# kennethsoh/IE-ACHE

Measured on AMD Instinct MI355X. Metric: bootstrapped gate ops/sec; encrypted 32-bit MUL/sec, higher is better.
Workload: dtype int32; 1 GPU; 16-bit ADD, batch 4096 ciphertext pairs, 1xMI355X (level-batched bootstraps); circuit=add16, batch_per_gpu=4096, bootstraps_per_expr=80, levels=48, params=n=630 N=1024 k=1 l=3 Bgbit=7 ks_t=8 ks_basebit=2, parallelism=batch-sharded x1, kernel=w1x64-radix8-onelimb, overlap_streams=2, rccl_ranks=0

## Files before the change

ie-ache_amd/__init__.py:

```python
from .evaluator import (
    CIRC_ADD, CIRC_SUB, CIRC_RSUB, CIRC_MUL, CIRC_MULADD, CIRC_ADD_KS, CIRC_SUB_KS, CIRC_RSUB_KS, CIRC_MUL_WALLACE,
    GATE_AND, GATE_XOR, GATE_OR, GATE_NAND, GATE_MUX, circ_chain,
    GATE_NOR, GATE_XNOR, GATE_ANDNY, GATE_ANDYN, GATE_ORNY, GATE_ORYN, GATE_TYPES, FALSE, TRUE, NOT, Netlist, CompiledNetlist,
    CircuitInfo, Context, IeacheError, Params, Stats, build_library, circuit_info, circuit_level_cap, circuit_simulate,
    default_params, device_count, debug_forward_path, lib, library_path,
    GATE_MAJ3, GATE_XOR3, CIRC_ADD_FA, CIRC_SUB_FA, CIRC_RSUB_FA, CIRC_MUL_FA, circuit_gate_count,
    PBS_NO_KEYSWITCH, PBS_TLWE_POLYS, PBS_ACCUMULATOR, PBS_MULTI_MAX_FACTORS, Group, GROUP_MAX_DEVICES, Job,
    TgswSet, Automaton, AUTOMATON_MAX_STATES, AUTOMATON_MAX_STEPS, automaton_tables, LUT_TREE_MAX_DEPTH, ROTATE_MAX_STEPS, LUT_READ_NO_KEYSWITCH,
    FFT_FORWARD_FORMS, FFT_INVERSE_FORMS, FFT_PAIRED_FORMS, TWIDDLE_ENTRIES,
)
from . import tools
from . import netlists
from . import automata
from . import programs
from .programs import WordProgram, Register, netlist_export
from .programs import FAMILY_REFERENCE, FAMILY_KOGGE_STONE, FAMILY_CARRY_SAVE, FAMILY_FULL_ADDER
from .compute import compute, compute_final, FAILURE_SIZE
```

ie-ache_amd/csrc/blind_rotate_w64.hip:

```cpp
#include "blind_rotate_w64.h"

#include <cstdio>
#include <algorithm>
#include <stdexcept>
#include <type_traits>
#include <vector>

#include "br_step.h"
#include "fft_probe.h"
#include "mix_plan.h"

namespace ieache {
namespace w64 {

using namespace dev;

namespace {

__global__ __launch_bounds__(64) void k_bk_to_spectrum_w64(const Torus32* bk_raw, double2* bkf) {
    __shared__ __align__(16) double2 sT[kTile];
    __shared__ __align__(16) double2 sTw[kTwElems];
    const int lane = threadIdx.x;
    build_twiddles(sTw, lane, 64);
    __syncthreads();
// ... 169 lines not shown
#pragma unroll 1
        for (int q = 1; q < L; q++) digit_row(q, std::false_type{});
        fft512_inverse_pair<true>(s[0], s[1], sT, lane, R);
#pragma unroll
        for (int r = 0; r < 8; r++) {
            double unused = 0.0;
            const uint32_t l0 = round_coef(s[0][r].x, untwist_gain(r), false, unused), l1 = round_coef(s[0][r].y, untwist_gain(r), false, unused);
            const uint32_t h0 = round_coef(s[1][r].x, untwist_gain(r), false, unused), h1 = round_coef(s[1][r].y, untwist_gain(r), false, unused);
            const int32_t j = 64 * r + lane;
            accw[j] = (int32_t)((uint32_t)accw[j] + l0 + (h0 << 16));
            accw[j + kM] = (int32_t)((uint32_t)accw[j + kM] + l1 + (h1 << 16));
        }
    }
    __syncthreads();
    finish_slice<128>(ext, item, acc, gacc, tid);
}


template <int L, int BGBIT, int GUARD, bool DIAG = false, int G = kW1Gates, int XLANE = 2>
__global__ __launch_bounds__(64 * G, 2) void k_blind_rotate_w1b(DevKeys K, const double2* __restrict__ bkf1,
                                                                       const uint16_t* __restrict__ st_bara, int32_t nb,
                                                                       int32_t* st_acc, int64_t items, int32_t i0, int32_t i1,
                                                                       Torus32* ext, unsigned* guard,
                                                                       const double2* __restrict__ gtw, unsigned long long* diag = nullptr) {
    extern __shared__ __align__(16) unsigned char smem[];
    int32_t* acc_all = reinterpret_cast<int32_t*>(smem);
    double2* sT_all = reinterpret_cast<double2*>(smem + (size_t)G * 2 * kN * 4);
    double2* sTw = sT_all + G * kTile;
    const int tid = threadIdx.x, lane = tid & 63;
    const int wave = __builtin_amdgcn_readfirstlane(tid >> 6);
    double2* sT = sT_all + wave * kTile;
    int32_t* acc = acc_all + wave * 2 * kN;
    const int64_t item = (int64_t)blockIdx.x * G + wave;
    static_assert(XLANE == 1 || XLANE == 2, "the forward transforms' lane-high transpose: v_cndmask pairs (1) or the exchange form (2)");
    using Roots = typename std::conditional<XLANE == 2, LaneRootsExchange, LaneRootsResident>::type;
    load_twiddles(sTw, gtw, tid, 64 * G);
    __syncthreads();
    if (item >= items) return;
    const Roots R = make_roots<Roots>(sTw, lane);
    const int plane = XLANE == 2 ? xl_pi(lane) : lane;
    const uint16_t* __restrict__ bara = st_bara + (size_t)item * nb;
    int32_t* gacc = st_acc + (size_t)item * 2 * kN;
    {
        const int4* src = reinterpret_cast<const int4*>(gacc);
        int4* dst = reinterpret_cast<int4*>(acc);
#pragma unroll
        for (int r = 0; r < 8; r++) dst[64 * r + lane] = src[64 * r + lane];
    }
    wave_sync();

    constexpr uint32_t halfBg = 1u << (BGBIT - 1);
    uint32_t dec_offset = 0;
#pragma unroll
    for (int q = 1; q <= L; q++) dec_offset += halfBg << (32 - q * BGBIT);
    float dev_maxf = 0.0f;
    constexpr int kRowBytes = 2 * kM * (int)sizeof(double2), kStepBytes = 2 * L * kRowBytes;
    const __amdgpu_buffer_rsrc_t bk_rsrc = bk_resource(bkf1, K.n, kStepBytes);
    const int lane16 = bk_lane_offset(lane);
    const unsigned char* accb = reinterpret_cast<const unsigned char*>(acc_all);
    const uint32_t pb0 = (uint32_t)wave * (2 * kN * 4);

    unsigned long long tsum[8] = {0, 0, 0, 0, 0, 0, 0, 0}, tlast = 0;
    if (DIAG) tlast = stamp();
    const int32_t my_a = lane_amounts(bara, i0, i1, lane);
#pragma unroll 1
    for (int32_t i = i0; i < i1; i++) {
        const int32_t a = __builtin_amdgcn_readlane(my_a, i - i0);
        if (a == 0) continue;
        const int bki = i * kStepBytes;
        double2 s[2][8];
        uint32_t v0[8], v1[8];
        double dev_max = 0.0;
        const uint32_t jb4 = ((uint32_t)(plane - a) & (2 * kN - 1)) << 2;
        auto decompose = [&](const uint32_t pb) {
            const int32_t* accp = reinterpret_cast<const int32_t*>(accb + pb);
            decompose_rotated(v0, v1, accb, accp, pb, jb4, plane, dec_offset);
        };
        auto digit_row = [&](const int sh, const int brow, auto first) {
            constexpr bool FIRST = decltype(first)::value;
            double2 x[8], bA[8], bB[8];
            auto request_a = [&]() { load_bk_block(bA, bk_rsrc, lane16, brow); };
            digits_to_double2<BGBIT>(x, v0, v1, sh);
            __builtin_amdgcn_sched_barrier(0);
            stamp_phase<DIAG>(tsum, tlast, 1);
            fft512_forward<true, XLANE>(x, sT, lane, R, request_a);
            stamp_phase<DIAG>(tsum, tlast, 2);
            load_bk_block(bB, bk_rsrc, lane16, brow + kRowBytes / 2);
            __builtin_amdgcn_sched_barrier(0);
#pragma unroll
            for (int k = 0; k < 8; k++) s[0][k] = mac<FIRST>(s[0][k], x[k], bA[k]);
#pragma unroll
            for (int k = 0; k < 8; k++) s[1][k] = mac<FIRST>(s[1][k], x[k], bB[k]);
            stamp_phase<DIAG>(tsum, tlast, 3);
        };
        decompose(pb0);
        stamp_phase<DIAG>(tsum, tlast, 0);
        digit_row(32 - BGBIT, bki, std::true_type{});
#pragma unroll 1
        for (int row = 1; row < L; row++) digit_row(32 - (row + 1) * BGBIT, bki + row * kRowBytes, std::false_type{});
        decompose(pb0 + 4096u);
        stamp_phase<DIAG>(tsum, tlast, 0);
#pragma unroll 1
        for (int row = L; row < 2 * L; row++) digit_row(32 - (row - L + 1) * BGBIT, bki + row * kRowBytes, std::false_type{});
        fft512_inverse_pair<true>(s[0], s[1], sT, lane, R);
        stamp_phase<DIAG>(tsum, tlast, 4);
#pragma unroll
        for (int c = 0; c < 2; c++) {
            uint32_t* accc = reinterpret_cast<uint32_t*>(acc) + c * kN;
#pragma unroll
            for (int r = 0; r < 8; r++) {
                const bool watched = GUARD == 1 || (GUARD == 2 && (r & 3) == 0);
                const uint32_t d0 = round_coef(s[c][r].x, untwist_gain(r), watched, dev_max), d1 = round_coef(s[c][r].y, untwist_gain(r), watched, dev_max);
                const int32_t j = 64 * r + lane;
                __hip_atomic_fetch_add(&accc[j], d0, __ATOMIC_RELAXED, __HIP_MEMORY_SCOPE_WAVEFRONT);
                __hip_atomic_fetch_add(&accc[j + kM], d1, __ATOMIC_RELAXED, __HIP_MEMORY_SCOPE_WAVEFRONT);
            }
        }
        if (GUARD) dev_maxf = fmaxf(dev_maxf, (float)dev_max);
        wave_sync();
        stamp_phase<DIAG>(tsum, tlast, 5);
    }
    if (DIAG && diag && lane == 0) {
#pragma unroll
        for (int t = 0; t < 8; t++) atomicAdd(&diag[(wave & 1) * 8 + t], tsum[t]);
    }
    int elane = lane;
    asm volatile("" : "+v"(elane));
    if (GUARD) publish_guard((double)dev_maxf, guard, elane);
    finish_slice<64>(ext, item, acc, gacc, elane);
}

template <int L, int BGBIT, int G = kW1Gates>
__global__ __launch_bounds__(64 * G, 2) void k_blind_rotate_x1(DevKeys K, const double2* __restrict__ bkf,
                                                                      const uint16_t* __restrict__ st_bara, int32_t nb,
                                                                      int32_t* st_acc, int64_t items, int32_t i0, int32_t i1,
                                                                      Torus32* ext, const double2* __restrict__ gtw) {
    extern __shared__ __align__(16) unsigned char smem[];
    int32_t* acc_all = reinterpret_cast<int32_t*>(smem);
    double2* sT_all = reinterpret_cast<double2*>(smem + (size_t)G * 2 * kN * 4);
    double2* sTw = sT_all + G * kTile;
    const int tid = threadIdx.x, lane = tid & 63;
    const int wave = __builtin_amdgcn_readfirstlane(tid >> 6);
    double2* sT = sT_all + wave * kTile;
    int32_t* acc = acc_all + wave * 2 * kN;
    const int64_t item = (int64_t)blockIdx.x * G + wave;
    load_twiddles(sTw, gtw, tid, 64 * G);
    __syncthreads();
    if (item >= items) return;
    const LaneRoots R = make_roots(sTw, lane);
    const uint16_t* __restrict__ bara = st_bara + (size_t)item * nb;
    int32_t* gacc = st_acc + (size_t)item * 2 * kN;
    {
        const int4* src = reinterpret_cast<const int4*>(gacc);
        int4* dst = reinterpret_cast<int4*>(acc);
#pragma unroll
        for (int r = 0; r < 8; r++) dst[64 * r + lane] = src[64 * r + lane];
    }
    wave_sync();

    constexpr uint32_t halfBg = 1u << (BGBIT - 1);
    uint32_t dec_offset = 0;
#pragma unroll
// ... 618 lines not shown
        char what[96];
        snprintf(what, sizeof what, "%s<%d,%d> (br_variant %d, %d gates per workgroup)", br_variant(v.number)->name, PS::L, PS::BGBIT, (int)v.number, v.gates);
        allow_dynamic_lds_once(grant, (const void*)kernel, v.allow, what);
    }
    hipLaunchKernelGGL(kernel, dim3((unsigned)((s.items + v.gates - 1) / v.gates)), dim3(v.threads == kTwoLWaves ? 128 * PS::L : v.threads),
                       v.lds(PS::L, s.nb, v.gates), s.stream, args...);
}
template <class PS, class... P>
static void launch_row(PS ps, const LaunchRow& v, const Slice& s, void (*kernel)(P...), typename as_is<P>::type... args) {
    launch_row_granted(ps, v, s, granted(v, PS::index), kernel, args...);
}
template <int XLANE>
static void go_w2(const LaunchRow& v, const Slice& s) {
    with_param_set(s.l, [&](auto ps) {
        launch_row(ps, v, s, k_blind_rotate_w2<ps.L, ps.BGBIT, XLANE>, s.K, s.t.bkf, s.st_bara, s.nb, s.st_acc, s.i0, s.i1, s.ext, s.t.twiddles);
    });
}
template <int G>
static void go_x1(const LaunchRow& v, const Slice& s) {
    with_param_set(s.l, [&](auto ps) {
        launch_row(ps, v, s, k_blind_rotate_x1<ps.L, ps.BGBIT, G>, s.K, s.t.bkf, s.st_bara, s.nb, s.st_acc, s.items, s.i0, s.i1, s.ext, s.t.twiddles);
    });
}
template <bool DIAG, int LIMBS>
static void go_wide(const LaunchRow& v, const Slice& s) {
    with_param_set(s.l, [&](auto ps) {
        launch_row(ps, v, s, k_blind_rotate_wide<ps.L, ps.BGBIT, DIAG, LIMBS>, s.K, LIMBS == 2 ? s.t.bkf : s.t.bkf1, s.st_bara, s.nb, s.st_acc,
                   s.i0, s.i1, s.ext, DIAG ? s.t.diag : nullptr, s.t.twiddles, LIMBS == 2 ? nullptr : s.t.guard);
    });
}
template <int GUARD, bool DIAG = false, int G = kW1Gates>
static void go_w1b(const LaunchRow& v, const Slice& s) {
    with_param_set(s.l, [&](auto ps) {
        constexpr int XL = (DIAG && ps.L == 2) ? 1 : 2;
        if constexpr (GUARD == 2 && !DIAG) {
            if (probe::w1b_forward_path() == 1) {
                static LdsGrant partner;
                launch_row_granted(ps, v, s, partner, k_blind_rotate_w1b<ps.L, ps.BGBIT, GUARD, DIAG, G, 1>, s.K, s.t.bkf1, s.st_bara, s.nb, s.st_acc,
                                   s.items, s.i0, s.i1, s.ext, s.t.guard, s.t.twiddles, nullptr);
                return;
            }
        }
        launch_row(ps, v, s, k_blind_rotate_w1b<ps.L, ps.BGBIT, GUARD, DIAG, G, XL>, s.K, s.t.bkf1, s.st_bara, s.nb, s.st_acc, s.items, s.i0, s.i1,
                   s.ext, s.t.guard, s.t.twiddles, DIAG ? s.t.diag : nullptr);
    });
}
template <int GUARD>
static void go_w2r(const LaunchRow& v, const Slice& s) {
    with_param_set(s.l, [&](auto ps) {
        launch_row(ps, v, s, k_blind_rotate_w2r<ps.L, ps.BGBIT, GUARD>, s.K, s.t.bkf1, s.st_bara, s.nb, s.st_acc, s.i0, s.i1, s.ext, s.t.guard, s.t.twiddles);
    });
}
template <int GUARD>
static void go_w4r(const LaunchRow& v, const Slice& s) {
    with_param_set(s.l, [&](auto ps) {
        launch_row(ps, v, s, k_blind_rotate_w4r<ps.L, ps.BGBIT, GUARD>, s.K, s.t.bkf1, s.st_bara, s.nb, s.st_acc, s.i0, s.i1, s.ext, s.t.guard, s.t.twiddles,
                   s.flip);
    });
}
template <int GUARD>
static void go_wide4(const LaunchRow& v, const Slice& s) {
    with_param_set(s.l, [&](auto ps) {
        launch_row(ps, v, s, k_blind_rotate_wide4<ps.L, ps.BGBIT, GUARD>, s.K, s.t.bkf1, s.st_bara, s.nb, s.st_acc, s.i0, s.i1, s.ext, s.t.guard, s.t.twiddles);
    });
}

constexpr size_t kAccBytes = (size_t)2 * kN * 4, kCuLds = 160 * 1024;
constexpr size_t lds_bytes_w1(int wg_gates) { return (size_t)(wg_gates * kTile + kTwElems) * sizeof(double2) + (size_t)wg_gates * 2 * kN * 4; }
static size_t lds_w1(int, int32_t, int gates) { return lds_bytes_w1(gates); }
static size_t lds_w2(int, int32_t, int) { return (size_t)(2 * kTile + kTwElems) * sizeof(double2) + kAccBytes; }
static size_t lds_w4(int, int32_t, int) { return (size_t)(4 * kTile + 2 * 8 * 64 + kTwElems) * sizeof(double2) + kAccBytes; }
static size_t lds_wide(int L, int32_t nb, int) { return (size_t)(2 * L * kTile + kTwElems) * sizeof(double2) + kAccBytes + (size_t)nb * 2; }
static size_t lds_wide4(int L, int32_t nb, int) { return (size_t)((2 * L + 4) * kTile + kTwElems) * sizeof(double2) + kAccBytes + (size_t)nb * 2; }

// ... 164 lines not shown
```

ie-ache_amd/csrc/br_step.h:

```cpp
#pragma once
#include "device_common.h"
#include "fft512.h"

namespace ieache {
namespace w64 {
namespace {

using namespace dev;

constexpr int kW1Gates = 4;
constexpr float kGuardLimit = 0.0625f;
__device__ __forceinline__ void publish_guard(double dev_max, unsigned* guard, int lane) {
    float m = (float)dev_max;
#pragma unroll
    for (int o = 32; o >= 1; o >>= 1) m = fmaxf(m, __shfl_xor(m, o, 64));
    if (lane == 0) {
        const unsigned bits = __float_as_uint(m);
        if (bits > __builtin_nontemporal_load(&guard[1])) atomicMax(&guard[1], bits);
        if (m > kGuardLimit) atomicAdd(&guard[0], 1u);
    }
}

template <int NT>
__device__ __forceinline__ void copy_acc(int32_t* to, const int32_t* from, int tid) {
    const int4* src = reinterpret_cast<const int4*>(from);
    int4* dst = reinterpret_cast<int4*>(to);
#pragma unroll
    for (int r = 0; r < 2 * kN / 4 / NT; r++) dst[NT * r + tid] = src[NT * r + tid];
}
template <int NT>
__device__ __forceinline__ void copy_acc_strided(int32_t* to, const int32_t* from, int tid) {
    const int4* src = reinterpret_cast<const int4*>(from);
    int4* dst = reinterpret_cast<int4*>(to);
    for (int idx = tid; idx < 2 * kN / 4; idx += NT) dst[idx] = src[idx];
}
template <int NT>
__device__ __forceinline__ void finish_slice(Torus32* ext, int64_t item, const int32_t* acc, int32_t* gacc, int tid) {
    if (ext) {
        Torus32* u = ext + (size_t)item * (kN + 4);
        for (int32_t j = tid; j <= kN; j += NT)
            u[j] = j == 0 ? acc[0] : (j == kN ? acc[kN] : (int32_t)(0u - (uint32_t)acc[kN - j]));
    } else {
        const int4* src = reinterpret_cast<const int4*>(acc);
        int4* dst = reinterpret_cast<int4*>(gacc);
#pragma unroll
        for (int r = 0; r < 2 * kN / 4 / NT; r++) dst[NT * r + tid] = src[NT * r + tid];
    }
}

__device__ __forceinline__ int32_t lane_amounts(const uint16_t* __restrict__ bara, int32_t i, int32_t i1, int lane) {
    return (i + lane < i1) ? (int32_t)bara[i + lane] : 0;
}

__device__ __forceinline__ __amdgpu_buffer_rsrc_t bk_resource(const double2* bkf, int32_t n, int step_bytes) {
    return __builtin_amdgcn_make_buffer_rsrc(const_cast<double2*>(bkf), (short)0, n * step_bytes, 0x00020000);
}
__device__ __forceinline__ int bk_lane_offset(int lane) { return lane * (int)sizeof(double2); }

template <int L, int BGBIT>
__device__ __forceinline__ uint32_t decomposition_offset() {
    constexpr uint32_t halfBg = 1u << (BGBIT - 1);
    uint32_t dec_offset = 0;
#pragma unroll
    for (int q = 1; q <= L; q++) dec_offset += halfBg << (32 - q * BGBIT);
    return dec_offset;
}
template <int BGBIT>
__device__ __forceinline__ int32_t signed_digit(uint32_t v, int sh) {
    return __builtin_amdgcn_sbfe((int32_t)v, sh, BGBIT);
}
template <int BGBIT>
__device__ __forceinline__ void digits_to_double2(double2 (&x)[8], const uint32_t (&v0)[8], const uint32_t (&v1)[8], int sh) {
#pragma unroll
    for (int r = 0; r < 8; r++) {
        const int32_t e0 = signed_digit<BGBIT>(v0[r], sh), e1 = signed_digit<BGBIT>(v1[r], sh);
        x[r] = make_double2((double)e0, (double)e1);
    }
}

__device__ __forceinline__ void decompose_rotated(uint32_t (&v0)[8], uint32_t (&v1)[8], const unsigned char* accb, const int32_t* accp,
                                                  uint32_t pb, uint32_t jb4, int lane, uint32_t dec_offset) {
#pragma unroll
    for (int r = 0; r < 8; r++) {
        const uint32_t t = jb4 + 256u * r;
        const uint32_t o0 = (t & 4092u) | pb, o1 = o0 ^ 2048u;
        const int32_t m0 = __builtin_amdgcn_sbfe((int32_t)t, 12, 1), m1 = __builtin_amdgcn_sbfe((int32_t)(t + 2048u), 12, 1);
        const uint32_t rv0 = *reinterpret_cast<const uint32_t*>(accb + o0), rv1 = *reinterpret_cast<const uint32_t*>(accb + o1);
        const uint32_t pv0 = (uint32_t)accp[64 * r + lane], pv1 = (uint32_t)accp[64 * r + lane + kM];
        v0[r] = ((rv0 ^ (uint32_t)m0) + ((dec_offset - pv0) - (uint32_t)m0)) ^ dec_offset;
        v1[r] = ((rv1 ^ (uint32_t)m1) + ((dec_offset - pv1) - (uint32_t)m1)) ^ dec_offset;
    }
}

template <bool FIRST>
__device__ __forceinline__ double2 mac(double2 s, double2 x, double2 b) {
    return FIRST ? cmulx<false>(x, b) : make_double2(fma(x.x, b.x, fma(-x.y, b.y, s.x)), fma(x.x, b.y, fma(x.y, b.x, s.y)));
}
template <bool FIRST>
__device__ __forceinline__ void mac_row(double2 (&s)[8], const double2 (&x)[8], const double2 (&b)[8]) {
#pragma unroll
    for (int k = 0; k < 8; k++) s[k] = mac<FIRST>(s[k], x[k], b[k]);
}

template <int BGBIT, bool FIRST>
__device__ __forceinline__ void digit_row_two_limb(double2 (&s)[4][8], const uint32_t (&v0)[8], const uint32_t (&v1)[8], int sh,
                                                   __amdgpu_buffer_rsrc_t bk_rsrc, int lane16, int brow, double2* sT, int lane, const LaneRoots& R) {
    constexpr int kBlockBytes = kM * (int)sizeof(double2);
    double2 x[8], bA[8], bB[8];
    digits_to_double2<BGBIT>(x, v0, v1, sh);
    __builtin_amdgcn_sched_barrier(0);
    auto req = [&]() { load_bk_block(bA, bk_rsrc, lane16, brow); };
    fft512_forward<true, 1, decltype(req), true>(x, sT, lane, R, req);
    load_bk_block(bB, bk_rsrc, lane16, brow + kBlockBytes);
    __builtin_amdgcn_sched_barrier(0);
    mac_row<FIRST>(s[0], x, bA);
    __builtin_amdgcn_sched_barrier(0);
    load_bk_block(bA, bk_rsrc, lane16, brow + 2 * kBlockBytes);
    __builtin_amdgcn_sched_barrier(0);
    mac_row<FIRST>(s[1], x, bB);
    __builtin_amdgcn_sched_barrier(0);
    load_bk_block(bB, bk_rsrc, lane16, brow + 3 * kBlockBytes);
    __builtin_amdgcn_sched_barrier(0);
    mac_row<FIRST>(s[2], x, bA);
    mac_row<FIRST>(s[3], x, bB);
}
// ... 52 lines not shown
```

ie-ache_amd/csrc/capi.cpp:

```cpp
#include "../../include/ieache.h"

#include <cerrno>
#include <cstdio>
#include <cstdlib>
#include <cstring>
#include <initializer_list>
#include <memory>
#include <mutex>
#include <new>
#include <string>
#include <vector>

#include "br_plan.h"
#include "circuit.h"
#include "circuit_cache.h"
#include "cloud_run.h"
#include "cmux.h"
#include "codec.h"
#include "daemon.h"
#include "evaluator.h"
#include "fft_probe.h"
#include "group.h"
#include "group_run.h"
#include "mix_plan.h"
// ... 1371 lines not shown
}

int ieache_debug_twiddles(ieache_ctx* ctx, int which, double* out) {
    return guarded([&] {
        if (!ctx || !out) return fail(IEACHE_EINVAL, "null argument");
        ctx->eval->debug_twiddles(which, out);
        return 0;
    });
}

int ieache_debug_fft512(ieache_ctx* ctx, int form, size_t count, const double* in, double* out) {
    return guarded([&] {
        if (!ctx || !in || !out) return fail(IEACHE_EINVAL, "null argument");
        ctx->eval->debug_fft512(form, count, in, out);
        return 0;
    });
}

int ieache_debug_spectrum(ieache_ctx* ctx, int which, size_t first, size_t count, double* out) {
    return guarded([&] {
        if (!ctx || !out) return fail(IEACHE_EINVAL, "null argument");
        ctx->eval->debug_spectrum(which, first, count, out);
        return 0;
    });
}

int ieache_debug_forward_path(int xlane) {
    return guarded([&] {
        probe::set_w1b_forward_path(xlane);
        return 0;
    });
}

struct ieache_group {
    std::unique_ptr<DeviceGroup> g;
    bool precheck = true;
    ieache_ctx* member(size_t m) const { return g->member(m); }
    size_t size() const { return g->size(); }
};

extern "C++" {
namespace {
struct MemberFailure {
    size_t member;
    int rc;
    std::string message;
};
template <class Call>
int group_call(ieache_group* grp, size_t count, ieache_stats* stats, Call&& call) {
    for (size_t m = 0; stats && m < grp->size(); m++) memset(&stats[m], 0, sizeof stats[m]);
    if (count == 0) return call(grp->member(0), (size_t)0, (size_t)0, stats);
    try {
        run_sliced(grp->size(), count, [&](size_t m, size_t first, size_t rows) {
            const int rc = call(grp->member(m), first, rows, stats ? stats + m : nullptr);
            if (rc < 0) throw MemberFailure{m, rc, ieache_last_error()};
        });
    } catch (const MemberFailure& f) {
        return fail(f.rc, grp->g->member_label(f.member) + f.message);
    }
    g_err.clear();
    return 0;
}
template <class Make>
ieache_group* make_group(Make&& make) {
    ieache_group* grp = nullptr;
    guarded([&] {
// ... 719 lines not shown
```

ie-ache_amd/csrc/fft_probe.h:

```cpp
#pragma once
#include <hip/hip_runtime.h>

#include <cstddef>

namespace ieache {
namespace probe {

constexpr int kForms = 8;
constexpr int kFirstInverseForm = 5, kFirstPairedForm = 6;
constexpr size_t kTransformElems = 512;
constexpr size_t kTwiddleElems = 576;

const char* form_refusal(int form, size_t count);
void run_fft512(int form, size_t count, const double2* d_in, double2* d_out, const double2* d_tw, hipStream_t stream);
void build_twiddles_in_wave(double2* d_out, hipStream_t stream);

void set_w1b_forward_path(int xlane);
int w1b_forward_path();

}
}
```

ie-ache_amd/csrc/fft_probe.hip:

```cpp
#include "fft_probe.h"

#include <atomic>
#include <cstdlib>
#include <stdexcept>

#include "evaluator.h"
#include "fft512.h"

namespace ieache {
namespace probe {

using namespace w64;

namespace {

constexpr int kWaves = 4;
static_assert(kTwiddleElems == (size_t)kTwElems && kTransformElems == (size_t)kM, "fft_probe.h restates tw_roots.h / fft512.h");

struct HookLoad {
    const double2* src;
    double2* dst;
    __device__ __forceinline__ void operator()() const { *dst = *src; }
};

// ... 77 lines not shown
}

const char* form_refusal(int form, size_t count) {
    if (form < 0 || form >= kForms) return "debug_fft512: unknown form (0 .. 7: csrc/fft_probe.h)";
    if (count < 1 || count > ((size_t)1 << 20)) return "debug_fft512: count must lie in 1 .. 2^20";
    if (form >= kFirstPairedForm && count % 2 != 0) return "debug_fft512: a paired form takes an even count";
    return nullptr;
}

void run_fft512(int form, size_t count, const double2* d_in, double2* d_out, const double2* d_tw, hipStream_t stream) {
    if (const char* why = form_refusal(form, count)) throw std::invalid_argument(why);
    const int64_t units = (int64_t)(form >= kFirstPairedForm ? count / 2 : count);
    double2* d_hook = nullptr;
    if (form >= 2 && form < kFirstInverseForm) HIP_CHECK(hipMalloc((void**)&d_hook, (size_t)units * 64 * sizeof(double2)));
    switch (form) {
        case 0: launch_form<0>(units, d_in, d_out, d_tw, d_hook, stream); break;
        case 1: launch_form<1>(units, d_in, d_out, d_tw, d_hook, stream); break;
        case 2: launch_form<2>(units, d_in, d_out, d_tw, d_hook, stream); break;
        case 3: launch_form<3>(units, d_in, d_out, d_tw, d_hook, stream); break;
        case 4: launch_form<4>(units, d_in, d_out, d_tw, d_hook, stream); break;
        case 5: launch_form<5>(units, d_in, d_out, d_tw, d_hook, stream); break;
        case 6: launch_form<6>(units, d_in, d_out, d_tw, d_hook, stream); break;
        default: launch_form<7>(units, d_in, d_out, d_tw, d_hook, stream); break;
    }
    const hipError_t launched = hipGetLastError();
    const hipError_t done = hipStreamSynchronize(stream);
    if (d_hook) (void)hipFree(d_hook);
    HIP_CHECK(launched);
    HIP_CHECK(done);
}

static int forward_path_at_start() {
    const char* e = getenv("IEACHE_W1B_FORWARD");
    return e && e[0] == '1' && !e[1] ? 1 : 2;
}
static std::atomic<int> g_w1b_forward_path{forward_path_at_start()};
void set_w1b_forward_path(int xlane) {
    if (xlane != 1 && xlane != 2) throw std::invalid_argument("debug_forward_path: 1 (v_cndmask pairs) or 2 (the exchange form, the default)");
    g_w1b_forward_path.store(xlane, std::memory_order_relaxed);
}
int w1b_forward_path() { return g_w1b_forward_path.load(std::memory_order_relaxed); }

void build_twiddles_in_wave(double2* d_out, hipStream_t stream) {
    hipLaunchKernelGGL(k_probe_build_twiddles, dim3(1), dim3(64), 0, stream, d_out);
    HIP_CHECK(hipGetLastError());
}

}
}
```

ie-ache_amd/evaluator.py:

```python
import ctypes as C
import os
import subprocess
import sys

import numpy as np

_PKG = os.path.dirname(os.path.abspath(__file__))
_LIB = None

CIRC_ADD, CIRC_SUB, CIRC_RSUB, CIRC_MUL, CIRC_MULADD = 1, 2, 3, 4, 5
CIRC_ADD_KS, CIRC_SUB_KS, CIRC_RSUB_KS = 6, 7, 8
CIRC_MUL_WALLACE = 9
GATE_AND, GATE_XOR, GATE_OR, GATE_NAND, GATE_MUX = 0, 1, 2, 3, 4
GATE_NOR, GATE_XNOR, GATE_ANDNY, GATE_ANDYN, GATE_ORNY, GATE_ORYN = 5, 6, 7, 8, 9, 10
GATE_TYPES = 11
LUT_TREE_MAX_DEPTH = 12
ROTATE_MAX_STEPS = 64
LUT_READ_NO_KEYSWITCH = 1
PBS_MULTI_MAX_FACTORS = 64
PBS_NO_KEYSWITCH = 1
PBS_TLWE_POLYS = 4
PBS_ACCUMULATOR = 8
GATE_MAJ3, GATE_XOR3 = 32, 33
CIRC_ADD_FA, CIRC_SUB_FA, CIRC_RSUB_FA, CIRC_MUL_FA = 16, 17, 18, 19
# ... 222 lines not shown
    jp = C.POINTER(Job)
    L.ieache_prepare_jobs.argtypes = [vp, jp, C.c_size_t]
    L.ieache_eval_jobs.argtypes = [vp, jp, C.c_size_t, sp]
    L.ieache_eval_jobs_device.argtypes = [vp, jp, C.c_size_t, sp]
    L.ieache_group_eval_jobs.argtypes = [vp, jp, C.c_size_t, sp]
    ip = C.POINTER(C.c_int)
    L.ieache_group_create.restype = vp
    L.ieache_group_create.argtypes = [C.c_char_p, ip, C.c_int]
    L.ieache_group_create_raw.restype = vp
    L.ieache_group_create_raw.argtypes = [pp, i32p, i32p, ip, C.c_int]
    L.ieache_group_destroy.restype = None
    L.ieache_group_destroy.argtypes = [vp]
    L.ieache_group_size.argtypes = [vp]
    L.ieache_group_device.argtypes = [vp, C.c_int]
    L.ieache_group_ctx.restype = vp
    L.ieache_group_ctx.argtypes = [vp, C.c_int]
    L.ieache_group_set_option.argtypes = [vp, C.c_char_p, C.c_int64]
    L.ieache_group_prepare_batch.argtypes = [vp, C.c_int, C.c_int, C.c_size_t]
    L.ieache_group_eval_batch.argtypes = [vp, C.c_int, C.c_int, C.c_size_t, i32p, i32p, sp]
    L.ieache_group_prepare_netlist.argtypes = [vp, vp, C.c_size_t]
    L.ieache_group_eval_netlist.argtypes = [vp, vp, C.c_size_t, i32p, i32p, sp]
    L.ieache_group_gates.argtypes = [vp, C.c_int, C.c_size_t, i32p, i32p, i32p, sp]
    L.ieache_group_gates3.argtypes = [vp, C.c_int, C.c_size_t, i32p, i32p, i32p, i32p, sp]
    L.ieache_group_mux.argtypes = [vp, C.c_size_t, i32p, i32p, i32p, i32p, sp]
    L.ieache_group_pbs.argtypes = [vp, C.c_size_t, i32p, i32p, C.c_int32, i32p, i32p, C.c_int, sp]
    L.ieache_group_pbs_multi.argtypes = [vp, C.c_size_t, i32p, i32p, C.c_int32, i32p, i32p, C.c_int32, i32p, i32p, C.c_int, sp]
    L.ieache_debug_blind_rotate.argtypes = [vp, C.c_size_t, i32p, i32p, C.c_int32]
    L.ieache_debug_keyswitch.argtypes = [vp, C.c_size_t, i32p, i32p]
    f64p = C.POINTER(C.c_double)
    L.ieache_debug_twiddles.argtypes = [vp, C.c_int, f64p]
    L.ieache_debug_fft512.argtypes = [vp, C.c_int, C.c_size_t, f64p, f64p]
    L.ieache_debug_spectrum.argtypes = [vp, C.c_int, C.c_size_t, C.c_size_t, f64p]
    L.ieache_debug_forward_path.argtypes = [C.c_int]
    L.ieache_keygen_raw.argtypes = [pp, u32p, C.c_int, i32p, i32p, i32p, i32p]
    L.ieache_keygen_files.argtypes = [C.c_char_p, pp, u32p, C.c_int, u32p, C.c_int]
    L.ieache_encrypt_bits.argtypes = [pp, i32p, u8p, C.c_size_t, C.c_uint64, i32p]
    L.ieache_decrypt_bits.argtypes = [pp, i32p, i32p, C.c_size_t, u8p]
    L.ieache_read_secret_key.argtypes = [C.c_char_p, pp, i32p, i32p]
    L.ieache_read_cloud_key.argtypes = [C.c_char_p, pp, i32p, i32p]
    L.ieache_write_cloud_key.argtypes = [C.c_char_p, pp, i32p, i32p]
    L.ieache_write_secret_key.argtypes = [C.c_char_p, pp, i32p, i32p, i32p, i32p]
    L.ieache_read_samples.argtypes = [C.c_char_p, C.c_int32, C.c_size_t, C.c_size_t, i32p]
    L.ieache_write_samples.argtypes = [C.c_char_p, C.c_int32, C.c_size_t, i32p, C.c_int]
    L.ieache_alice.argtypes = [C.c_char_p, C.c_char_p, C.c_char_p, C.c_int, C.c_uint32, C.c_uint32, u32p, C.c_uint64]
    L.ieache_verif.argtypes = [C.c_char_p, C.c_char_p, C.c_char_p, u32p, u32p, u32p]
    L.ieache_serve.restype = C.c_int64
    L.ieache_serve.argtypes = [C.c_char_p, C.c_char_p, C.c_char_p, C.c_int, C.c_int64]
    L.ieache_serve_devices.restype = C.c_int64
    L.ieache_serve_devices.argtypes = [C.c_char_p, C.c_char_p, C.c_char_p, C.POINTER(C.c_int), C.c_int, C.c_int64]
    L.ieache_debug_mix_plan.argtypes = [C.c_int, C.c_int, C.c_int64, C.c_int, C.c_int, C.POINTER(C.c_int)]
    L.ieache_shard_slice.argtypes = [C.c_size_t, C.c_size_t, C.c_size_t, C.POINTER(C.c_size_t), C.POINTER(C.c_size_t)]
    L.ieache_client_ping.argtypes = [C.c_char_p]
    L.ieache_client_run_dir.argtypes = [C.c_char_p, C.c_char_p]
    L.ieache_client_run_data.argtypes = [C.c_char_p, C.c_int, vp, C.c_size_t, vp, C.c_size_t, C.POINTER(C.c_size_t)]
    L.ieache_client_shutdown.argtypes = [C.c_char_p]
    _LIB = L
    return L


def check(rc):
    if rc < 0:
        raise IeacheError(rc, lib().ieache_last_error().decode())
    return rc


def _i32(a):
# ... 50 lines not shown
            nl, in_lwe = job
            info = nl.info()
            arr[i].netlist = nl.h
        else:
            kind, bits, in_lwe = job
            info = circuit_info(kind, bits, fold)
            arr[i].kind, arr[i].bits = int(kind), int(bits)
        in_lwe = np.ascontiguousarray(in_lwe, dtype=np.int32)
        batch = in_lwe.shape[0]
        assert in_lwe.shape == (batch, info.n_inputs, n_words), in_lwe.shape
        out = np.zeros((batch, info.n_outputs, n_words), dtype=np.int32)
        arr[i].batch = batch
        arr[i].in_lwe = in_lwe.ctypes.data
        arr[i].out_lwe = out.ctypes.data
        ins.append(in_lwe)
        outs.append(out)
    return arr, ins, outs


def default_params():
    p = Params()
    lib().ieache_default_params(C.byref(p))
    return p


def device_count():
    return lib().ieache_device_count()


def debug_forward_path(xlane):
    check(lib().ieache_debug_forward_path(xlane))


def circuit_info(kind, bits, fold=False, level_cap=0):
    info = CircuitInfo()
    check(lib().ieache_circuit_info_get_cap(kind, bits, int(fold), int(level_cap), C.byref(info)))
    return info


def circuit_gate_count(kind, bits, gate_type, fold=False):
    return check(lib().ieache_circuit_gate_count(kind, bits, int(fold), int(gate_type)))


def circuit_level_cap(kind, bits, batch, resident_workgroups=1024, fold=False):
    return check(lib().ieache_circuit_level_cap(kind, bits, int(fold), int(batch), int(resident_workgroups)))


def circuit_simulate(kind, bits, in_bits, fold=False, level_cap=0):
    info = circuit_info(kind, bits, fold)
    in_bits = np.ascontiguousarray(in_bits, dtype=np.uint8)
    assert in_bits.shape == (info.n_inputs,)
    out = np.zeros(info.n_outputs, dtype=np.uint8)
    check(lib().ieache_circuit_simulate_cap(kind, bits, int(fold), int(level_cap), in_bits.ctypes.data_as(C.POINTER(C.c_uint8)),
                                            out.ctypes.data_as(C.POINTER(C.c_uint8))))
    return out


class Netlist:

    def __init__(self, n_inputs):
        self.n_inputs = int(n_inputs)
        self._gates = []

    def input(self, i):
        if not 0 <= i < self.n_inputs:
            raise IndexError("netlist input %d of %d" % (i, self.n_inputs))
# ... 813 lines not shown
```

include/ieache.h:

```cpp
#ifndef IEACHE_H
#define IEACHE_H
#include <stddef.h>
#include <stdint.h>

#ifdef __cplusplus
extern "C" {
#endif

#define IEACHE_EINVAL (-22)
#define IEACHE_EIO (-5)
#define IEACHE_ENODEV (-19)
#define IEACHE_ENOMEM (-12)

typedef struct ieache_params {
    int32_t n, N, k, l, Bgbit, ks_t, ks_basebit;
    double lwe_alpha_min, lwe_alpha_max, tlwe_alpha_min, tlwe_alpha_max;
} ieache_params;

void ieache_default_params(ieache_params* out);

typedef struct ieache_stats {
    double total_ms;
    double blind_rotate_ms;
    double keyswitch_ms;
// ... 201 lines not shown
#define IEACHE_WOP_EQ 17
#define IEACHE_WOP_SELECT 18
#define IEACHE_FAMILY_REFERENCE 0
#define IEACHE_FAMILY_KOGGE_STONE 1
#define IEACHE_FAMILY_CARRY_SAVE 2
#define IEACHE_FAMILY_FULL_ADDER 3
#define IEACHE_PROGRAM_FOLD 2
#define IEACHE_WORD_MAX_WIDTH 512
typedef struct ieache_word_instr {
    int32_t op;
    int32_t family;
    int32_t width;
    int32_t a, b, c;
    int32_t imm0, imm1;
    int32_t first, count;
} ieache_word_instr;
typedef struct ieache_word_arg {
    int32_t reg, shift;
} ieache_word_arg;
ieache_netlist* ieache_program_compile(const ieache_word_instr* instrs, size_t n_instrs, const ieache_word_arg* args, size_t n_args,
                                       const uint32_t* const_words, size_t n_const_words, const int32_t* outputs, size_t n_outputs,
                                       int flags);
int64_t ieache_netlist_export(const ieache_netlist* nl, ieache_net_gate* gates, size_t cap, int32_t* outputs, size_t out_cap);

int ieache_circuit_simulate(int kind, int bits, const uint8_t* in_bits, uint8_t* out_bits);
int ieache_circuit_simulate_ex(int kind, int bits, int fold_constants, const uint8_t* in_bits, uint8_t* out_bits);

int ieache_debug_blind_rotate(ieache_ctx* ctx, size_t count, const int32_t* x, int32_t* acc, int32_t steps);
int ieache_debug_keyswitch(ieache_ctx* ctx, size_t count, const int32_t* u, int32_t* out);
int ieache_debug_twiddles(ieache_ctx* ctx, int which, double* out);
int ieache_debug_fft512(ieache_ctx* ctx, int form, size_t count, const double* in, double* out);
int ieache_debug_spectrum(ieache_ctx* ctx, int which, size_t first, size_t count, double* out);
int ieache_debug_forward_path(int xlane);
int ieache_debug_mix_plan(int cus, int n, int64_t gates, int s1, int ratio_x100, int out[9]);

int ieache_ctx_set_packing_key(ieache_ctx* ctx, int32_t pk_t, int32_t pk_basebit, const int32_t* pk );
int ieache_debug_pack_plan(const ieache_ctx* ctx, size_t groups, int32_t m, int64_t out[4]);
int ieache_pack_device(ieache_ctx* ctx, size_t groups, int32_t m, int32_t spread, int32_t shift,
                       const int32_t* d_rows , int32_t* d_out , ieache_stats* stats);
int ieache_pack(ieache_ctx* ctx, size_t groups, int32_t m, int32_t spread, int32_t shift,
                const int32_t* rows , int32_t* out , ieache_stats* stats);

#define IEACHE_LUT_TREE_MAX_DEPTH 12
typedef struct ieache_tgsw ieache_tgsw;
ieache_tgsw* ieache_tgsw_prepare(ieache_ctx* ctx, const int32_t* samples , size_t n);
ieache_tgsw* ieache_tgsw_prepare_device(ieache_ctx* ctx, const int32_t* d_samples , size_t n);
void ieache_tgsw_free(ieache_tgsw* set);
int ieache_cmux(ieache_ctx* ctx, const ieache_tgsw* set, size_t count, const int32_t* sel_of ,
                const int32_t* d1 , const int32_t* d0 , int32_t* out , ieache_stats* stats);
int ieache_cmux_device(ieache_ctx* ctx, const ieache_tgsw* set, size_t count, const int32_t* d_sel_of, const int32_t* d_d1, const int32_t* d_d0,
                       int32_t* d_out, ieache_stats* stats);
int ieache_lut_tree(ieache_ctx* ctx, const ieache_tgsw* set, size_t count, int32_t depth, const int32_t* sel_of ,
                    const int32_t* tables , int32_t n_tables, const int32_t* table_of ,
                    int32_t* out , ieache_stats* stats);
int ieache_lut_tree_device(ieache_ctx* ctx, const ieache_tgsw* set, size_t count, int32_t depth, const int32_t* d_sel_of, const int32_t* d_tables,
                           int32_t n_tables, const int32_t* d_table_of, int32_t* d_out, ieache_stats* stats);
int ieache_tlwe_extract(ieache_ctx* ctx, size_t count, const int32_t* tlwe , const int32_t* coef_of ,
                        int32_t* u , ieache_stats* stats);
int ieache_tlwe_extract_device(ieache_ctx* ctx, size_t count, const int32_t* d_tlwe, const int32_t* d_coef_of,
                               int32_t* d_u , ieache_stats* stats);
int ieache_debug_cmux_plan(const ieache_ctx* ctx, size_t count, int32_t depth, int64_t out[4]);

int ieache_lut_scatter(ieache_ctx* ctx, const ieache_tgsw* set, size_t count, int32_t depth, const int32_t* sel_of ,
                       const int32_t* values , const int32_t* mem ,
                       int32_t* out , ieache_stats* stats);
int ieache_lut_scatter_device(ieache_ctx* ctx, const ieache_tgsw* set, size_t count, int32_t depth, const int32_t* d_sel_of,
// ... 133 lines not shown
```

Before: 217,200 gate ops/s.

## Store blind-rotate accumulators in a bank-folded LDS layout with planned rotated gathers

Adds a folded (XOR-swizzled) layout for the per-wave accumulator in shared memory to the w1b blind-rotate kernel. The rotated-gather addresses are precomputed once per step and reused by both polynomials' decompositions, and reads are batched. The load, atomic-add write-back and the finish routine are all remapped to the same fold. The aim is to cut LDS bank conflicts and address arithmetic in the decomposition, at the risk of extra index math and mismatched fold mappings. The default for l=3 with the guard is path 2, now folded; a path 3 keeps the natural layout.

```diff
diff --git a/ie-ache_amd/__init__.py b/ie-ache_amd/__init__.py
--- a/ie-ache_amd/__init__.py
+++ b/ie-ache_amd/__init__.py
@@ -3,7 +3,7 @@
     GATE_AND, GATE_XOR, GATE_OR, GATE_NAND, GATE_MUX, circ_chain,
     GATE_NOR, GATE_XNOR, GATE_ANDNY, GATE_ANDYN, GATE_ORNY, GATE_ORYN, GATE_TYPES, FALSE, TRUE, NOT, Netlist, CompiledNetlist,
     CircuitInfo, Context, IeacheError, Params, Stats, build_library, circuit_info, circuit_level_cap, circuit_simulate,
-    default_params, device_count, debug_forward_path, lib, library_path,
+    default_params, device_count, debug_forward_path, debug_w1b_path, lib, library_path,
     GATE_MAJ3, GATE_XOR3, CIRC_ADD_FA, CIRC_SUB_FA, CIRC_RSUB_FA, CIRC_MUL_FA, circuit_gate_count,
     PBS_NO_KEYSWITCH, PBS_TLWE_POLYS, PBS_ACCUMULATOR, PBS_MULTI_MAX_FACTORS, Group, GROUP_MAX_DEVICES, Job,
     TgswSet, Automaton, AUTOMATON_MAX_STATES, AUTOMATON_MAX_STEPS, automaton_tables, LUT_TREE_MAX_DEPTH, ROTATE_MAX_STEPS, LUT_READ_NO_KEYSWITCH,
diff --git a/ie-ache_amd/csrc/acc_fold.h b/ie-ache_amd/csrc/acc_fold.h
--- /dev/null
+++ b/ie-ache_amd/csrc/acc_fold.h
@@ -0,0 +1,25 @@
+#pragma once
+
+#include <cstdint>
+
+#ifndef IEACHE_HD
+#ifdef __HIPCC__
+#define IEACHE_HD __device__ __forceinline__
+#else
+#define IEACHE_HD inline
+#endif
+#endif
+
+namespace ieache {
+namespace w64 {
+
+IEACHE_HD constexpr uint32_t acc_fold(uint32_t d) { return d ^ (((d >> 5) & 1u) << 4); }
+IEACHE_HD constexpr uint32_t acc_fold4(uint32_t q) { return q ^ (((q >> 3) & 1u) << 2); }
+IEACHE_HD constexpr uint32_t acc_fold_bytes(uint32_t b) { return b ^ ((b >> 1) & 64u); }
+
+IEACHE_HD constexpr uint32_t acc_fold_step_offset(uint32_t own, uint32_t half, uint32_t gate_4a) {
+    return acc_fold_bytes(((own ^ (half & 64u)) - gate_4a) & 8188u);
+}
+
+}
+}
diff --git a/ie-ache_amd/csrc/blind_rotate_w64.hip b/ie-ache_amd/csrc/blind_rotate_w64.hip
--- a/ie-ache_amd/csrc/blind_rotate_w64.hip
+++ b/ie-ache_amd/csrc/blind_rotate_w64.hip
@@ -225,20 +225,22 @@
     double2* sT = sT_all + wave * kTile;
     int32_t* acc = acc_all + wave * 2 * kN;
     const int64_t item = (int64_t)blockIdx.x * G + wave;
-    static_assert(XLANE == 1 || XLANE == 2, "the forward transforms' lane-high transpose: v_cndmask pairs (1) or the exchange form (2)");
-    using Roots = typename std::conditional<XLANE == 2, LaneRootsExchange, LaneRootsResident>::type;
+    static_assert(XLANE >= 1 && XLANE <= 3, "v_cndmask pairs (1), the exchange form on folded accumulators (2) or on natural ones (3)");
+    constexpr int FX = XLANE == 1 ? 1 : 2;
+    constexpr bool FOLD = XLANE == 2;
+    using Roots = typename std::conditional<FX == 2, LaneRootsExchange, LaneRootsResident>::type;
     load_twiddles(sTw, gtw, tid, 64 * G);
     __syncthreads();
     if (item >= items) return;
     const Roots R = make_roots<Roots>(sTw, lane);
-    const int plane = XLANE == 2 ? xl_pi(lane) : lane;
+    const int plane = FX == 2 ? xl_pi(lane) : lane;
     const uint16_t* __restrict__ bara = st_bara + (size_t)item * nb;
     int32_t* gacc = st_acc + (size_t)item * 2 * kN;
     {
         const int4* src = reinterpret_cast<const int4*>(gacc);
         int4* dst = reinterpret_cast<int4*>(acc);
 #pragma unroll
-        for (int r = 0; r < 8; r++) dst[64 * r + lane] = src[64 * r + lane];
+        for (int r = 0; r < 8; r++) dst[64 * r + (FOLD ? (int)acc_fold4((uint32_t)lane) : lane)] = src[64 * r + lane];
     }
     wave_sync();
 
@@ -252,6 +254,8 @@
     const int lane16 = bk_lane_offset(lane);
     const unsigned char* accb = reinterpret_cast<const unsigned char*>(acc_all);
     const uint32_t pb0 = (uint32_t)wave * (2 * kN * 4);
+    const int flane = FOLD ? (int)acc_fold((uint32_t)lane) : lane;
+    const uint32_t accl0 = FOLD ? lds_address(acc) : 0u, ownl0 = accl0 + 4u * acc_fold((uint32_t)plane);
 
     unsigned long long tsum[8] = {0, 0, 0, 0, 0, 0, 0, 0}, tlast = 0;
     if (DIAG) tlast = stamp();
@@ -264,10 +268,25 @@
         double2 s[2][8];
         uint32_t v0[8], v1[8];
         double dev_max = 0.0;
-        const uint32_t jb4 = ((uint32_t)(plane - a) & (2 * kN - 1)) << 2;
-        auto decompose = [&](const uint32_t pb) {
-            const int32_t* accp = reinterpret_cast<const int32_t*>(accb + pb);
-            decompose_rotated(v0, v1, accb, accp, pb, jb4, plane, dec_offset);
+        uint32_t jb4;
+        if constexpr (FOLD) {
+            uint32_t half;
+            asm volatile("v_lshrrev_b32 %0, 1, %1" : "=v"(half) : "v"(ownl0));
+            jb4 = acc_fold_step_offset(ownl0, half, accl0 + 4u * (uint32_t)a);
+        } else {
+            jb4 = ((uint32_t)(plane - a) & (2 * kN - 1)) << 2;
+        }
+        RotatedGather gather;
+        if constexpr (FOLD) plan_rotated_gather(gather, accl0, jb4, dec_offset);
+        auto decompose = [&](auto poly) {
+            constexpr int POLY = decltype(poly)::value;
+            if constexpr (FOLD) {
+                decompose_planned<POLY, 4>(v0, v1, gather, ownl0, dec_offset);
+            } else {
+                const uint32_t pb = pb0 + 4096u * POLY;
+                const int32_t* accp = reinterpret_cast<const int32_t*>(accb + pb);
+                decompose_rotated(v0, v1, accb, accp, pb, jb4, plane, dec_offset);
+            }
         };
         auto digit_row = [&](const int sh, const int brow, auto first) {
             constexpr bool FIRST = decltype(first)::value;
@@ -276,7 +295,7 @@
             digits_to_double2<BGBIT>(x, v0, v1, sh);
             __builtin_amdgcn_sched_barrier(0);
             stamp_phase<DIAG>(tsum, tlast, 1);
-            fft512_forward<true, XLANE>(x, sT, lane, R, request_a);
+            fft512_forward<true, FX>(x, sT, lane, R, request_a);
             stamp_phase<DIAG>(tsum, tlast, 2);
             load_bk_block(bB, bk_rsrc, lane16, brow + kRowBytes / 2);
             __builtin_amdgcn_sched_barrier(0);
@@ -286,12 +305,12 @@
             for (int k = 0; k < 8; k++) s[1][k] = mac<FIRST>(s[1][k], x[k], bB[k]);
             stamp_phase<DIAG>(tsum, tlast, 3);
         };
-        decompose(pb0);
+        decompose(std::integral_constant<int, 0>{});
         stamp_phase<DIAG>(tsum, tlast, 0);
         digit_row(32 - BGBIT, bki, std::true_type{});
 #pragma unroll 1
         for (int row = 1; row < L; row++) digit_row(32 - (row + 1) * BGBIT, bki + row * kRowBytes, std::false_type{});
-        decompose(pb0 + 4096u);
+        decompose(std::integral_constant<int, 1>{});
         stamp_phase<DIAG>(tsum, tlast, 0);
 #pragma unroll 1
         for (int row = L; row < 2 * L; row++) digit_row(32 - (row - L + 1) * BGBIT, bki + row * kRowBytes, std::false_type{});
@@ -304,7 +323,7 @@
             for (int r = 0; r < 8; r++) {
                 const bool watched = GUARD == 1 || (GUARD == 2 && (r & 3) == 0);
                 const uint32_t d0 = round_coef(s[c][r].x, untwist_gain(r), watched, dev_max), d1 = round_coef(s[c][r].y, untwist_gain(r), watched, dev_max);
-                const int32_t j = 64 * r + lane;
+                const int32_t j = 64 * r + flane;
                 __hip_atomic_fetch_add(&accc[j], d0, __ATOMIC_RELAXED, __HIP_MEMORY_SCOPE_WAVEFRONT);
                 __hip_atomic_fetch_add(&accc[j + kM], d1, __ATOMIC_RELAXED, __HIP_MEMORY_SCOPE_WAVEFRONT);
             }
@@ -320,7 +339,10 @@
     int elane = lane;
     asm volatile("" : "+v"(elane));
     if (GUARD) publish_guard((double)dev_maxf, guard, elane);
-    finish_slice<64>(ext, item, acc, gacc, elane);
+    if constexpr (FOLD)
+        finish_slice_folded<64>(ext, item, acc, gacc, elane);
+    else
+        finish_slice<64>(ext, item, acc, gacc, elane);
 }
 
 template <int L, int BGBIT, int G = kW1Gates>
@@ -1005,14 +1027,16 @@
 template <int GUARD, bool DIAG = false, int G = kW1Gates>
 static void go_w1b(const LaunchRow& v, const Slice& s) {
     with_param_set(s.l, [&](auto ps) {
-        constexpr int XL = (DIAG && ps.L == 2) ? 1 : 2;
+        constexpr int XL = (DIAG && ps.L == 2) ? 1 : (GUARD != 2 && ps.L == 2) ? 3 : 2;
         if constexpr (GUARD == 2 && !DIAG) {
-            if (probe::w1b_forward_path() == 1) {
+            auto partner_build = [&](auto xl) {
                 static LdsGrant partner;
-                launch_row_granted(ps, v, s, partner, k_blind_rotate_w1b<ps.L, ps.BGBIT, GUARD, DIAG, G, 1>, s.K, s.t.bkf1, s.st_bara, s.nb, s.st_acc,
-                                   s.items, s.i0, s.i1, s.ext, s.t.guard, s.t.twiddles, nullptr);
-                return;
-            }
+                launch_row_granted(ps, v, s, partner, k_blind_rotate_w1b<ps.L, ps.BGBIT, GUARD, DIAG, G, decltype(xl)::value>, s.K, s.t.bkf1, s.st_bara, s.nb,
+                                   s.st_acc, s.items, s.i0, s.i1, s.ext, s.t.guard, s.t.twiddles, nullptr);
+            };
+            const int path = probe::w1b_forward_path();
+            if (path == 1) return partner_build(std::integral_constant<int, 1>{});
+            if (path == 3) return partner_build(std::integral_constant<int, 3>{});
         }
         launch_row(ps, v, s, k_blind_rotate_w1b<ps.L, ps.BGBIT, GUARD, DIAG, G, XL>, s.K, s.t.bkf1, s.st_bara, s.nb, s.st_acc, s.items, s.i0, s.i1,
                    s.ext, s.t.guard, s.t.twiddles, DIAG ? s.t.diag : nullptr);
diff --git a/ie-ache_amd/csrc/br_step.h b/ie-ache_amd/csrc/br_step.h
--- a/ie-ache_amd/csrc/br_step.h
+++ b/ie-ache_amd/csrc/br_step.h
@@ -1,4 +1,5 @@
 #pragma once
+#include "acc_fold.h"
 #include "device_common.h"
 #include "fft512.h"
 
@@ -47,6 +48,23 @@
         for (int r = 0; r < 2 * kN / 4 / NT; r++) dst[NT * r + tid] = src[NT * r + tid];
     }
 }
+template <int NT>
+__device__ __forceinline__ void finish_slice_folded(Torus32* ext, int64_t item, const int32_t* acc, int32_t* gacc, int tid) {
+    if (ext) {
+        Torus32* u = ext + (size_t)item * (kN + 4);
+#pragma unroll 1
+        for (int32_t j = tid; j <= kN; j += NT) {
+            const bool end = j == 0 || j == kN;
+            const int32_t w = acc[end ? (uint32_t)j : acc_fold((uint32_t)(kN - j))];
+            u[j] = end ? w : (int32_t)(0u - (uint32_t)w);
+        }
+    } else {
+        const int4* src = reinterpret_cast<const int4*>(acc);
+        int4* dst = reinterpret_cast<int4*>(gacc);
+#pragma unroll
+        for (int r = 0; r < 2 * kN / 4 / NT; r++) dst[NT * r + tid] = src[NT * r + (int)acc_fold4((uint32_t)tid)];
+    }
+}
 
 __device__ __forceinline__ int32_t lane_amounts(const uint16_t* __restrict__ bara, int32_t i, int32_t i1, int lane) {
     return (i + lane < i1) ? (int32_t)bara[i + lane] : 0;
@@ -91,6 +109,55 @@
         v1[r] = ((rv1 ^ (uint32_t)m1) + ((dec_offset - pv1) - (uint32_t)m1)) ^ dec_offset;
     }
 }
+using LdsWord = const __attribute__((address_space(3))) uint32_t;
+__device__ __forceinline__ uint32_t lds_address(const void* p) {
+    return (uint32_t)(uintptr_t)(const __attribute__((address_space(3))) void*)p;
+}
+__device__ __forceinline__ uint32_t lds_word(uint32_t address) { return *reinterpret_cast<LdsWord*>((uintptr_t)address); }
+struct RotatedGather {
+    uint32_t a0[8];
+    int32_t m0[8], m1[8];
+    uint32_t k0[8], k1[8];
+};
+__device__ __forceinline__ void plan_rotated_gather(RotatedGather& g, uint32_t accl, uint32_t jb4, uint32_t dec_offset) {
+#pragma unroll
+    for (int r = 0; r < 8; r++) {
+        const uint32_t t = jb4 + 256u * r;
+        g.a0[r] = (t & 4092u) | accl;
+        g.m0[r] = __builtin_amdgcn_sbfe((int32_t)t, 12, 1), g.m1[r] = __builtin_amdgcn_sbfe((int32_t)(t + 2048u), 12, 1);
+        asm("" : "+v"(g.m0[r]));
+        asm("" : "+v"(g.m1[r]));
+        g.k0[r] = dec_offset - (uint32_t)g.m0[r], g.k1[r] = dec_offset - (uint32_t)g.m1[r];
+    }
+}
+template <int POLY, int BATCH>
+__device__ __forceinline__ void decompose_planned(uint32_t (&v0)[8], uint32_t (&v1)[8], const RotatedGather& g, uint32_t ownl, uint32_t dec_offset) {
+    static_assert(BATCH == 2 || BATCH == 4 || BATCH == 8, "registers per batch of reads");
+    constexpr uint32_t pb = 4096u * POLY;
+#pragma unroll
+    for (int h = 0; h < 8; h += BATCH) {
+        uint32_t rv0[BATCH], rv1[BATCH], pv0[BATCH], pv1[BATCH];
+#pragma unroll
+        for (int q = 0; q < BATCH; q++) {
+            const int r = h + q;
+            uint32_t a1;
+            if constexpr (POLY == 0)
+                asm("v_xor_b32 %0, 0x800, %1 ; polynomial 0" : "=v"(a1) : "v"(g.a0[r]));
+            else
+                asm("v_xor_b32 %0, 0x800, %1 ; polynomial 1" : "=v"(a1) : "v"(g.a0[r]));
+            rv0[q] = lds_word(g.a0[r] + pb), rv1[q] = lds_word(a1 + pb);
+            pv0[q] = lds_word(ownl + 256u * r + pb), pv1[q] = lds_word(ownl + 256u * r + 4u * kM + pb);
+        }
+        __builtin_amdgcn_sched_barrier(0);
+#pragma unroll
+        for (int q = 0; q < BATCH; q++) {
+            const int r = h + q;
+            v0[r] = ((rv0[q] ^ (uint32_t)g.m0[r]) + (g.k0[r] - pv0[q])) ^ dec_offset;
+            v1[r] = ((rv1[q] ^ (uint32_t)g.m1[r]) + (g.k1[r] - pv1[q])) ^ dec_offset;
+        }
+        __builtin_amdgcn_sched_barrier(0);
+    }
+}
 
 template <bool FIRST>
 __device__ __forceinline__ double2 mac(double2 s, double2 x, double2 b) {
diff --git a/ie-ache_amd/csrc/capi.cpp b/ie-ache_amd/csrc/capi.cpp
--- a/ie-ache_amd/csrc/capi.cpp
+++ b/ie-ache_amd/csrc/capi.cpp
@@ -1427,6 +1427,13 @@
     });
 }
 
+int ieache_debug_w1b_path(int path) {
+    return guarded([&] {
+        probe::set_w1b_path(path);
+        return 0;
+    });
+}
+
 struct ieache_group {
     std::unique_ptr<DeviceGroup> g;
     bool precheck = true;
diff --git a/ie-ache_amd/csrc/fft_probe.h b/ie-ache_amd/csrc/fft_probe.h
--- a/ie-ache_amd/csrc/fft_probe.h
+++ b/ie-ache_amd/csrc/fft_probe.h
@@ -16,6 +16,7 @@
 void build_twiddles_in_wave(double2* d_out, hipStream_t stream);
 
 void set_w1b_forward_path(int xlane);
+void set_w1b_path(int path);
 int w1b_forward_path();
 
 }
diff --git a/ie-ache_amd/csrc/fft_probe.hip b/ie-ache_amd/csrc/fft_probe.hip
--- a/ie-ache_amd/csrc/fft_probe.hip
+++ b/ie-ache_amd/csrc/fft_probe.hip
@@ -133,12 +133,17 @@
 
 static int forward_path_at_start() {
     const char* e = getenv("IEACHE_W1B_FORWARD");
-    return e && e[0] == '1' && !e[1] ? 1 : 2;
+    return e && (e[0] == '1' || e[0] == '3') && !e[1] ? e[0] - '0' : 2;
 }
 static std::atomic<int> g_w1b_forward_path{forward_path_at_start()};
 void set_w1b_forward_path(int xlane) {
     if (xlane != 1 && xlane != 2) throw std::invalid_argument("debug_forward_path: 1 (v_cndmask pairs) or 2 (the exchange form, the default)");
     g_w1b_forward_path.store(xlane, std::memory_order_relaxed);
+}
+void set_w1b_path(int path) {
+    if (path < 1 || path > 3)
+        throw std::invalid_argument("debug_w1b_path: 1 (v_cndmask pairs), 2 (the exchange form on folded accumulators, the default) or 3 (on natural ones)");
+    g_w1b_forward_path.store(path, std::memory_order_relaxed);
 }
 int w1b_forward_path() { return g_w1b_forward_path.load(std::memory_order_relaxed); }
 
diff --git a/ie-ache_amd/evaluator.py b/ie-ache_amd/evaluator.py
--- a/ie-ache_amd/evaluator.py
+++ b/ie-ache_amd/evaluator.py
@@ -278,6 +278,7 @@
     L.ieache_debug_fft512.argtypes = [vp, C.c_int, C.c_size_t, f64p, f64p]
     L.ieache_debug_spectrum.argtypes = [vp, C.c_int, C.c_size_t, C.c_size_t, f64p]
     L.ieache_debug_forward_path.argtypes = [C.c_int]
+    L.ieache_debug_w1b_path.argtypes = [C.c_int]
     L.ieache_keygen_raw.argtypes = [pp, u32p, C.c_int, i32p, i32p, i32p, i32p]
     L.ieache_keygen_files.argtypes = [C.c_char_p, pp, u32p, C.c_int, u32p, C.c_int]
     L.ieache_encrypt_bits.argtypes = [pp, i32p, u8p, C.c_size_t, C.c_uint64, i32p]
@@ -394,6 +395,10 @@
     check(lib().ieache_debug_forward_path(xlane))
 
 
+def debug_w1b_path(path):
+    check(lib().ieache_debug_w1b_path(path))
+
+
 def circuit_info(kind, bits, fold=False, level_cap=0):
     info = CircuitInfo()
     check(lib().ieache_circuit_info_get_cap(kind, bits, int(fold), int(level_cap), C.byref(info)))
diff --git a/include/ieache.h b/include/ieache.h
--- a/include/ieache.h
+++ b/include/ieache.h
@@ -257,6 +257,7 @@
 int ieache_debug_fft512(ieache_ctx* ctx, int form, size_t count, const double* in, double* out);
 int ieache_debug_spectrum(ieache_ctx* ctx, int which, size_t first, size_t count, double* out);
 int ieache_debug_forward_path(int xlane);
+int ieache_debug_w1b_path(int path);
 int ieache_debug_mix_plan(int cus, int n, int64_t gates, int s1, int ratio_x100, int out[9]);
 
 int ieache_ctx_set_packing_key(ieache_ctx* ctx, int32_t pk_t, int32_t pk_basebit, const int32_t* pk );
```

New measurement: 219,000 gate ops/s (median of 6 runs). No clear change (+0.8%).
